# cxy1997/3D_adapt_auto_driving

Hardware: AMD Instinct MI355X
Metric: KITTI scenes/s end-to-end eval_rcnn (joint RPN+RCNN, synthetic 16384-pt scenes) (higher is better)
Workload: dtype f32; 1 GPU; BASELINE.json configs[2]: full PointRCNN RPN+RCNN inference, default.yaml shapes, random-init weights, batch=8 synthetic KITTI scenes x 16384 pts per GPU per step; scene=synth.scenes (SURVEY 8d: uniform clutter + ground + 10 dense cars), parallelism=scene-sharded x1, one final all_gather of detections, detections_gathered=652455, batch_slots=14, look_ahead=12, steps_per_launch=2

## Files before the change

3d_adapt_auto_driving_amd/csrc/packed_layer.hip:

```cpp
#include "common.hpp"
#include <cstdlib>
#include "segmax.hpp"

namespace prcnn {

unsigned int *next_ticket(hipStream_t st);

typedef float f32x4 __attribute__((ext_vector_type(4)));
constexpr int PL_ROWS = 64;
constexpr int PL_LD = 128 + 4;

constexpr int PL_MAX_BATCH = 4;
struct PLProblem {
    const unsigned int *hdr; long rows_host; int K, N; const float *A; long lda; const float *W; const float *bias; int do_relu;
    float *out; long ldo; const unsigned int *rowinfo; const int *tilecloud; int m, out_col, n_store;
    int lds_pool;
    const float *addG; const int *addIdx; const float *addW; int add_n, add_m; long add_ldg;
};
struct PLBatch { PLProblem p[PL_MAX_BATCH]; };
struct PGProblem {
    int n, c1; const unsigned int *hdr; const float4 *rowdxyz; const float4 *P; const float4 *wxyz; const unsigned int *rowinfo;
    const int *tilecloud; float4 *out;
};
struct PGBatch { PGProblem p[PL_MAX_BATCH]; };

__global__ __launch_bounds__(256) void packed_gather_affine_kernel(const PGBatch bt)
{
    const PGProblem &pb = bt.p[blockIdx.z];
    const int n = pb.n, c1 = pb.c1;
    const unsigned int *__restrict__ hdr = pb.hdr;
    const float4 *__restrict__ rowdxyz = pb.rowdxyz;
    const float4 *__restrict__ P = pb.P;
    const float4 *__restrict__ wxyz = pb.wxyz;
    const unsigned int *__restrict__ rowinfo = pb.rowinfo;
    const int *__restrict__ tilecloud = pb.tilecloud;
    float4 *__restrict__ out = pb.out;
    const long t = blockIdx.x;
    if (t >= (long)hdr[0]) return;
    const int cloud = tilecloud[t];
    const int q4 = c1 / 4;
    const long pbase = (long)cloud * n;
    for (int e = threadIdx.x; e < PL_ROWS * q4; e += 256) {
        const int row = e / q4, q = e - row * q4;
        const int k = (int)(rowinfo[t * PL_ROWS + row] & 0xffffu);
        const float4 d = rowdxyz[t * PL_ROWS + row];
        const float dx = d.x, dy = d.y, dz = d.z;
        const float4 base = P[(pbase + k) * q4 + q];
        const float4 wx = wxyz[q], wy = wxyz[q4 + q], wz = wxyz[2 * q4 + q];
        const float4 v = affine_relu4(base, wx, wy, wz, dx, dy, dz);
        out[(t * PL_ROWS + row) * q4 + q] = v;
    }
}

#define PL_LOAD_W(dst, kk)                                                                              \
    _Pragma("unroll") for (int s = 0; s < 64; ++s)                                                      \
        dst[s] = __uint_as_float(__builtin_amdgcn_raw_buffer_load_b32(wrs, lane_off, (unsigned int)((kk) + s) * row_bytes, 0));
#define PL_LOAD_A(dst, kk)                                                                              \
    _Pragma("unroll") for (int i = 0; i < 8; ++i) {                                                     \
        long g = t * PL_ROWS + r0 + 8 * i;                                                              \
        if (g >= rows) g = rows - 1;    \
        dst[i] = *reinterpret_cast<const f32x4 *>(A + g * lda + (kk) + 4 * chunk);                     \
    }
#define PL_STORE_A(src)                                                                                 \
    _Pragma("unroll") for (int i = 0; i < 8; ++i)                                                       \
        *reinterpret_cast<f32x4 *>(tile + (r0 + 8 * i) * PL_LD + 4 * chunk) = src[i];
#define PL_VM_DRAIN __builtin_amdgcn_s_waitcnt(0x0F70);
#define PL_GROUP_MFMA_HEAD(wf)                                                                          \
    acc0 = __builtin_amdgcn_mfma_f32_32x32x2f32(a0.x, wf[4 * g + 0], acc0, 0, 0, 0);                    \
    acc1 = __builtin_amdgcn_mfma_f32_32x32x2f32(a1.x, wf[4 * g + 0], acc1, 0, 0, 0);
#define PL_GROUP_MFMA_TAIL(wf)                                                                          \
    acc0 = __builtin_amdgcn_mfma_f32_32x32x2f32(a0.y, wf[4 * g + 1], acc0, 0, 0, 0);                    \
    acc1 = __builtin_amdgcn_mfma_f32_32x32x2f32(a1.y, wf[4 * g + 1], acc1, 0, 0, 0);                    \
    acc0 = __builtin_amdgcn_mfma_f32_32x32x2f32(a0.z, wf[4 * g + 2], acc0, 0, 0, 0);                    \
    acc1 = __builtin_amdgcn_mfma_f32_32x32x2f32(a1.z, wf[4 * g + 2], acc1, 0, 0, 0);                    \
    acc0 = __builtin_amdgcn_mfma_f32_32x32x2f32(a0.w, wf[4 * g + 3], acc0, 0, 0, 0);                    \
    acc1 = __builtin_amdgcn_mfma_f32_32x32x2f32(a1.w, wf[4 * g + 3], acc1, 0, 0, 0);
#define PL_STAGE(T, wf)                                                                                 \
    {                                                                                                   \
        const float *a0p = (T) + j * PL_LD + 64 * h, *a1p = (T) + (32 + j) * PL_LD + 64 * h;            \
        f32x4 a0 = *reinterpret_cast<const f32x4 *>(a0p);                                               \
        f32x4 a1 = *reinterpret_cast<const f32x4 *>(a1p);                                               \
        _Pragma("unroll") for (int g = 0; g < 16; ++g) {                                                \
            f32x4 n0 = a0, n1 = a1;                                                                     \
            if (g < 15) {                                                                               \
                n0 = *reinterpret_cast<const f32x4 *>(a0p + 4 * (g + 1));                               \
                n1 = *reinterpret_cast<const f32x4 *>(a1p + 4 * (g + 1));                               \
            }                                                                                           \
            __builtin_amdgcn_sched_barrier(0);                                                          \
            PL_GROUP_MFMA_HEAD(wf)                                                                      \
            PL_GROUP_MFMA_TAIL(wf)                                                                      \
            a0 = n0; a1 = n1;                                                                           \
        }                                                                                               \
    }
#define PL_SADD(x, y) asm volatile("s_add_u32 %0, %0, %1" : "+s"(x) : "s"(y) : "scc");
#define PL_STAGE_PREFETCH_X(T, TN, wf, wn, kn, ARS, LOFF)                                               \
    {                                                                                                   \
        const float *a0p = (T) + j * PL_LD + 64 * h, *a1p = (T) + (32 + j) * PL_LD + 64 * h;            \
        f32x4 a0 = *reinterpret_cast<const f32x4 *>(a0p);                                               \
        f32x4 a1 = *reinterpret_cast<const f32x4 *>(a1p);                                               \
        f32x4 ar[8];                                                                                    \
// ... 39 lines not shown
            __builtin_amdgcn_sched_barrier(0);                                                          \
            PL_GROUP_MFMA_HEAD(wf)                                                                      \
            if (g < 8)                                                                                  \
                ar[g] = __builtin_bit_cast(f32x4, __builtin_amdgcn_raw_buffer_load_b128(                \
                    ars, a_lane, (soff) + (unsigned int)(8 * g) * a_row_bytes, 0));                     \
            else                                                                                        \
                *reinterpret_cast<f32x4 *>((TN) + (r0 + 8 * (g - 8)) * PL_LD + 4 * chunk) = ar[g - 8];  \
            __builtin_amdgcn_sched_barrier(0);                                                          \
            PL_GROUP_MFMA_TAIL(wf)                                                                      \
            a0 = n0_; a1 = n1_;                                                                         \
        }                                                                                               \
    }

template <bool SEGMAX>
__device__ __forceinline__ void pl_epilogue(const f32x16 &acc0, const f32x16 &acc1, float *tile, int *ctr, long t, long rows, int n0,
                                            const float *__restrict__ bias, int do_relu, float *__restrict__ out, long ldo,
                                            const unsigned int *__restrict__ rowinfo, const int *__restrict__ tilecloud, int m,
                                            int out_col, int n_store, int lds_pool, const PLProblem *add = nullptr)
{
    const int tid = threadIdx.x, lane = tid & 63, w = tid >> 6, j = lane & 31, h = lane >> 5;
    const int chunk = tid & 31, r0 = tid >> 5;
    const float bcol = bias[n0 + 32 * w + j];
    if constexpr (SEGMAX) {
        if (tid < PL_ROWS) {
            const unsigned int info = rowinfo[t * PL_ROWS + tid];
            ctr[tid] = tilecloud[t] * m + (int)(info >> 16);
        }
        __syncthreads();
        const int myc = ctr[lane], prevc = ctr[lane ? lane - 1 : 0];
        const unsigned long long start = __ballot(lane == 0 || myc != prevc);
        if (!lds_pool || __popcll(start) <= PK_LDS_MIN) {
            pk_segmented_max(acc0, acc1, ctr, start, h, out, (int)ldo, out_col + n0 + 32 * w + j, bcol);
        } else {
            const float4 bias4 = *reinterpret_cast<const float4 *>(bias + n0 + 4 * chunk);
            pk_park(acc0, acc1, tile, PL_LD, 32 * w + j, h);
            lds_barrier();
            pk_segmented_max_lds(tile, PL_LD, ctr, tid, out, (int)ldo, out_col + n0, bias4);
        }
    } else {
        const bool with_add = add && add->addG;
        __syncthreads();
#pragma unroll
        for (int r = 0; r < 16; ++r) {
            const int row = (r & 3) + 8 * (r >> 2) + 4 * h;
            const float v0 = acc0[r] + bcol, v1 = acc1[r] + bcol;
            tile[row * PL_LD + 32 * w + j] = (do_relu && !with_add) ? fmaxf(v0, 0.f) : v0;
            tile[(32 + row) * PL_LD + 32 * w + j] = (do_relu && !with_add) ? fmaxf(v1, 0.f) : v1;
        }
        __syncthreads();
#pragma unroll
        for (int i = 0; i < 8; ++i) {
            const int row = r0 + 8 * i;
            const long g = t * PL_ROWS + row;
            if (g < rows) {
                const int c0 = n0 + 4 * chunk;
                float4 v = *reinterpret_cast<const float4 *>(tile + row * PL_LD + 4 * chunk);
                if (with_add) {
                    const int *ix = add->addIdx + g * 3;
                    const float *wv = add->addW + g * 3;
                    const long cb = (g / add->add_n) * (long)add->add_m;
                    const float4 g0 = *reinterpret_cast<const float4 *>(add->addG + (cb + ix[0]) * add->add_ldg + c0);
                    const float4 g1 = *reinterpret_cast<const float4 *>(add->addG + (cb + ix[1]) * add->add_ldg + c0);
                    const float4 g2 = *reinterpret_cast<const float4 *>(add->addG + (cb + ix[2]) * add->add_ldg + c0);
                    const float w0 = wv[0], w1 = wv[1], w2 = wv[2];
                    v.x = __fadd_rn(v.x, __fadd_rn(__fadd_rn(__fmul_rn(w0, g0.x), __fmul_rn(w1, g1.x)), __fmul_rn(w2, g2.x)));
                    v.y = __fadd_rn(v.y, __fadd_rn(__fadd_rn(__fmul_rn(w0, g0.y), __fmul_rn(w1, g1.y)), __fmul_rn(w2, g2.y)));
                    v.z = __fadd_rn(v.z, __fadd_rn(__fadd_rn(__fmul_rn(w0, g0.z), __fmul_rn(w1, g1.z)), __fmul_rn(w2, g2.z)));
                    v.w = __fadd_rn(v.w, __fadd_rn(__fadd_rn(__fmul_rn(w0, g0.w), __fmul_rn(w1, g1.w)), __fmul_rn(w2, g2.w)));
                    if (do_relu) v = make_float4(fmaxf(v.x, 0.f), fmaxf(v.y, 0.f), fmaxf(v.z, 0.f), fmaxf(v.w, 0.f));
                }
                if (c0 + 4 <= n_store && (ldo & 3) == 0) {
                    *reinterpret_cast<float4 *>(out + g * ldo + c0) = v;
                } else {
                    const float e[4] = {v.x, v.y, v.z, v.w};
#pragma unroll
                    for (int q = 0; q < 4; ++q)
                        if (c0 + q < n_store) out[g * ldo + c0 + q] = e[q];
                }
            }
        }
    }
}

template <bool SEGMAX>
__global__ __launch_bounds__(256, 2) void packed_layer_kernel(
    const PLBatch bt)
{
    const PLProblem &pb = bt.p[blockIdx.z];
    const unsigned int *__restrict__ hdr = pb.hdr;
    const long rows_host = pb.rows_host;
    const int K = pb.K, N = pb.N;
    const float *__restrict__ A = pb.A;
    const long lda = pb.lda;
    const float *__restrict__ W = pb.W;
    const float *__restrict__ bias = pb.bias;
    const int do_relu = pb.do_relu;
    float *__restrict__ out = pb.out;
    const long ldo = pb.ldo;
    const unsigned int *__restrict__ rowinfo = pb.rowinfo;
    const int *__restrict__ tilecloud = pb.tilecloud;
    const int m = pb.m, out_col = pb.out_col, n_store = pb.n_store;
    __shared__ float tile[PL_ROWS * PL_LD];
    __shared__ int ctr[PL_ROWS];
    const long t = blockIdx.x;
    const long rows = hdr ? (long)hdr[0] * PL_ROWS : rows_host;
    const int n0 = blockIdx.y * 128;
    if (t * PL_ROWS >= rows || n0 >= n_store) return;
    const int tid = threadIdx.x, lane = tid & 63, w = tid >> 6, j = lane & 31, h = lane >> 5;
    const int chunk = tid & 31, r0 = tid >> 5;
    f32x16 acc0 = {0}, acc1 = {0};
    const __amdgpu_buffer_rsrc_t wrs = __builtin_amdgcn_make_buffer_rsrc((void *)W, 0, K * N * 4, 0x00020000);
    const unsigned int row_bytes = (unsigned int)N * 4u;
    const unsigned int lane_off = ((unsigned int)(64 * h) * (unsigned int)N + (unsigned int)(n0 + 32 * w + j)) * 4u;
    for (int k0 = 0; k0 < K; k0 += 128) {
        float wf[64];
        f32x4 ar[8];
        PL_LOAD_W(wf, k0)
        PL_LOAD_A(ar, k0)
        if (k0) __syncthreads();
        PL_STORE_A(ar)
        __syncthreads();
        PL_STAGE(tile, wf)
    }
    pl_epilogue<SEGMAX>(acc0, acc1, tile, ctr, t, rows, n0, bias, do_relu, out, ldo, rowinfo, tilecloud, m, out_col, n_store, pb.lds_pool, &pb);
}

template <bool SEGMAX>
__global__ __launch_bounds__(256, 2) void packed_layer_pipe_kernel(
    const PLBatch bt)
{
    const PLProblem &pb = bt.p[blockIdx.z];
    const unsigned int *__restrict__ hdr = pb.hdr;
    const long rows_host = pb.rows_host;
    const int K = pb.K, N = pb.N;
    const float *__restrict__ A = pb.A;
    const long lda = pb.lda;
    const float *__restrict__ W = pb.W;
    const float *__restrict__ bias = pb.bias;
    const int do_relu = pb.do_relu;
    float *__restrict__ out = pb.out;
    const long ldo = pb.ldo;
    const unsigned int *__restrict__ rowinfo = pb.rowinfo;
    const int *__restrict__ tilecloud = pb.tilecloud;
    const int m = pb.m, out_col = pb.out_col, n_store = pb.n_store;
    __shared__ float tiles[2 * PL_ROWS * PL_LD];
    __shared__ int ctr[PL_ROWS];
    const long t = blockIdx.x;
    const long rows = hdr ? (long)hdr[0] * PL_ROWS : rows_host;
    const int n0 = blockIdx.y * 128;
    if (t * PL_ROWS >= rows || n0 >= n_store) return;
    const int tid = threadIdx.x, lane = tid & 63, j = lane & 31, h = lane >> 5;
    const int w = __builtin_amdgcn_readfirstlane(tid >> 6);
    const int chunk = tid & 31, r0 = tid >> 5;
    f32x16 acc0 = {0}, acc1 = {0};
    const __amdgpu_buffer_rsrc_t wrs = __builtin_amdgcn_make_buffer_rsrc((void *)W, 0, K * N * 4, 0x00020000);
    const unsigned int row_bytes = (unsigned int)N * 4u;
    const unsigned int lane_off = ((unsigned int)(64 * h) * (unsigned int)N + (unsigned int)(n0 + 32 * w + j)) * 4u;
    const long left = rows - t * PL_ROWS;
    const unsigned int a_row_bytes = (unsigned int)lda * 4u;
    const __amdgpu_buffer_rsrc_t ars = __builtin_amdgcn_make_buffer_rsrc(
        (void *)(A + t * PL_ROWS * lda), 0, (int)((left < PL_ROWS ? left : PL_ROWS) * (long)a_row_bytes), 0x00020000);
    const unsigned int a_lane = (unsigned int)r0 * a_row_bytes + 16u * chunk;
    float wa[64], wb[64];
    {
        PL_LOAD_W(wa, 0)
#pragma unroll
        for (int i = 0; i < 8; ++i)
            *reinterpret_cast<f32x4 *>(tiles + (r0 + 8 * i) * PL_LD + 4 * chunk) =
                __builtin_bit_cast(f32x4, __builtin_amdgcn_raw_buffer_load_b128(ars, a_lane, (unsigned int)(8 * i) * a_row_bytes, 0));
    }
    const int np = K >> 7;
    for (int p = 0; p < np; ++p) {
        PL_VM_DRAIN
        lds_barrier();
        const float *T = tiles + (p & 1) * (PL_ROWS * PL_LD);
        float *TN = tiles + ((p + 1) & 1) * (PL_ROWS * PL_LD);
        if (p + 1 < np) {
            PL_STAGE_PREFETCH(T, TN, wa, wb, (p + 1) * 128)
#pragma unroll
            for (int s = 0; s < 64; ++s) wa[s] = wb[s];
        } else {
            PL_STAGE(T, wa)
        }
    }
    if constexpr (!SEGMAX) {
        if (n0 + 128 <= n_store && !pb.addG) {
            const float bcol = bias[n0 + 32 * w + j];
            const unsigned int o_row_bytes = (unsigned int)ldo * 4u;
            const __amdgpu_buffer_rsrc_t ors = __builtin_amdgcn_make_buffer_rsrc(
                (void *)(out + t * PL_ROWS * ldo), 0, (int)((left < PL_ROWS ? left : PL_ROWS) * (long)o_row_bytes), 0x00020000);
            const unsigned int o_lane = (unsigned int)(4 * h) * o_row_bytes + (unsigned int)(n0 + 32 * w + j) * 4u;
#pragma unroll
            for (int r = 0; r < 16; ++r) {
                const unsigned int so = (unsigned int)((r & 3) + 8 * (r >> 2)) * o_row_bytes;
                const float v0 = acc0[r] + bcol, v1 = acc1[r] + bcol;
                __builtin_amdgcn_raw_buffer_store_b32(__float_as_uint(do_relu ? fmaxf(v0, 0.f) : v0), ors, o_lane, so, 0);
                __builtin_amdgcn_raw_buffer_store_b32(__float_as_uint(do_relu ? fmaxf(v1, 0.f) : v1), ors, o_lane, so + 32u * o_row_bytes, 0);
            }
            return;
        }
    }
    pl_epilogue<SEGMAX>(acc0, acc1, tiles, ctr, t, rows, n0, bias, do_relu, out, ldo, rowinfo, tilecloud, m, out_col, n_store, pb.lds_pool, &pb);
}

template <bool ADD>
__global__ __launch_bounds__(256, 2) void packed_layer_persist_kernel(
    long rows, int K, int N, const float *__restrict__ A, long lda, const float *__restrict__ W, const float *__restrict__ bias,
    int do_relu, float *__restrict__ out, long ldo, unsigned int *__restrict__ ticket, const PLProblem addp)
{
    __shared__ float tiles[2 * PL_ROWS * PL_LD];
    __shared__ unsigned int s_item[2];
    const int tid = threadIdx.x, lane = tid & 63, j = lane & 31, h = lane >> 5;
    const int w = __builtin_amdgcn_readfirstlane(tid >> 6);
    const int chunk = tid & 31, r0 = tid >> 5;
    const unsigned int col_blocks = (unsigned int)(N >> 7);
    const unsigned int n_tiles = (unsigned int)((rows + PL_ROWS - 1) / PL_ROWS);
    const unsigned int n_items = n_tiles * col_blocks;
    const __amdgpu_buffer_rsrc_t wrs = __builtin_amdgcn_make_buffer_rsrc((void *)W, 0, K * N * 4, 0x00020000);
    const unsigned int row_bytes = (unsigned int)N * 4u;
    const unsigned int a_row_bytes = (unsigned int)lda * 4u;
    const unsigned int a_lane = (unsigned int)r0 * a_row_bytes + 16u * chunk;
    const int np = K >> 7;
    auto tile_rsrc = [&](unsigned int t) __attribute__((always_inline)) {
        const long left = rows - (long)t * PL_ROWS;
        return __builtin_amdgcn_make_buffer_rsrc((void *)(A + (long)t * PL_ROWS * lda), 0,
                                                 (int)((left < PL_ROWS ? left : PL_ROWS) * (long)a_row_bytes), 0x00020000);
    };
    auto loff = [&](unsigned int cb) __attribute__((always_inline)) {
        return ((unsigned int)(64 * h) * (unsigned int)N + (cb * 128u + (unsigned int)(32 * w + j))) * 4u;
    };
    unsigned int item = blockIdx.x;
    unsigned int t = item / col_blocks, cb = item - t * col_blocks;
    __amdgpu_buffer_rsrc_t ars = tile_rsrc(t);
    unsigned int lane_off = loff(cb);
    float wa[64], wb[64];
    {
        PL_LOAD_W(wa, 0)
#pragma unroll
        for (int i = 0; i < 8; ++i)
            *reinterpret_cast<f32x4 *>(tiles + (r0 + 8 * i) * PL_LD + 4 * chunk) =
                __builtin_bit_cast(f32x4, __builtin_amdgcn_raw_buffer_load_b128(ars, a_lane, (unsigned int)(8 * i) * a_row_bytes, 0));
    }
    int pp = 0;
    int slot = 1;
    PL_VM_DRAIN
    while (true) {
        f32x16 acc0 = {0}, acc1 = {0};
        unsigned int next = 0xffffffffu, tn = 0, cbn = 0, drawn = 0;
        const float bcol = bias[(int)cb * 128 + 32 * w + j];
        for (int p = 0; p < np; ++p, ++pp) {
            if (p > 0) {
                PL_VM_DRAIN
                if (p == 1 && tid == 0) s_item[slot] = drawn;
            }
            lds_barrier();
            if (p == 0 && tid == 0) drawn = gridDim.x + atomicAdd(ticket, 1u);
            const float *T = tiles + (pp & 1) * (PL_ROWS * PL_LD);
            float *TN = tiles + ((pp + 1) & 1) * (PL_ROWS * PL_LD);
            if (p + 1 < np) {
                PL_STAGE_PREFETCH(T, TN, wa, wb, (p + 1) * 128)
#pragma unroll
                for (int s2 = 0; s2 < 64; ++s2) wa[s2] = wb[s2];
            } else {
                next = s_item[slot];
                if (next < n_items) {
                    tn = next / col_blocks; cbn = next - tn * col_blocks;
                    const __amdgpu_buffer_rsrc_t ars_n = tile_rsrc(tn);
                    const unsigned int loff_n = loff(cbn);
                    PL_STAGE_PREFETCH_X(T, TN, wa, wb, 0, ars_n, loff_n)
#pragma unroll
                    for (int s2 = 0; s2 < 64; ++s2) wa[s2] = wb[s2];
                    PL_VM_DRAIN
                } else {
                    PL_STAGE(T, wa)
                }
            }
        }
        if constexpr (ADD) {
            float *Tlast = tiles + ((pp - 1) & 1) * (PL_ROWS * PL_LD);
            pl_epilogue<false>(acc0, acc1, Tlast, nullptr, (long)t, rows, (int)cb * 128, bias, do_relu, out, ldo, nullptr, nullptr, 0, 0, N, 0, &addp);
            __syncthreads();
        } else {
            const long left = rows - (long)t * PL_ROWS;
            const unsigned int o_row_bytes = (unsigned int)ldo * 4u;
            const __amdgpu_buffer_rsrc_t ors = __builtin_amdgcn_make_buffer_rsrc(
                (void *)(out + (long)t * PL_ROWS * ldo), 0, (int)((left < PL_ROWS ? left : PL_ROWS) * (long)o_row_bytes), 0x00020000);
            const unsigned int o_lane = (unsigned int)(4 * h) * o_row_bytes + (cb * 128u + (unsigned int)(32 * w + j)) * 4u;
#pragma unroll
            for (int r = 0; r < 16; ++r) {
                const unsigned int so = (unsigned int)((r & 3) + 8 * (r >> 2)) * o_row_bytes;
                const float v0 = acc0[r] + bcol, v1 = acc1[r] + bcol;
                __builtin_amdgcn_raw_buffer_store_b32(__float_as_uint(do_relu ? fmaxf(v0, 0.f) : v0), ors, o_lane, so, 0);
                __builtin_amdgcn_raw_buffer_store_b32(__float_as_uint(do_relu ? fmaxf(v1, 0.f) : v1), ors, o_lane, so + 32u * o_row_bytes, 0);
            }
        }
        if (next >= n_items) break;
        t = tn; cb = cbn;
        ars = tile_rsrc(t);
        lane_off = loff(cb);
        slot ^= 1;
    }
    if (tid == 0) ticket_release(ticket);
}

__global__ __launch_bounds__(256, 2) void packed_layer_stream_kernel(long rows, int N, const float *__restrict__ A, long lda,
                                                                     const float *__restrict__ W, const float *__restrict__ bias,
                                                                     int do_relu, float *__restrict__ out, long ldo, int n_store,
                                                                     const PLProblem addp )
{
    __shared__ float tiles[2 * PL_ROWS * PL_LD];
    const int tid = threadIdx.x, lane = tid & 63, j = lane & 31, h = lane >> 5;
    const int w = __builtin_amdgcn_readfirstlane(tid >> 6);
    const int chunk = tid & 31, r0 = tid >> 5;
    const int n0 = blockIdx.y * 128;
    const long ntiles = (rows + PL_ROWS - 1) / PL_ROWS;
    long t = blockIdx.x;
    if (t >= ntiles || n0 >= n_store) return;
    const __amdgpu_buffer_rsrc_t wrs = __builtin_amdgcn_make_buffer_rsrc((void *)W, 0, 128 * N * 4, 0x00020000);
    const unsigned int row_bytes = (unsigned int)N * 4u;
    const unsigned int lane_off = ((unsigned int)(64 * h) * (unsigned int)N + (unsigned int)(n0 + 32 * w + j)) * 4u;
    float wf[64];
    PL_LOAD_W(wf, 0)
    const unsigned int a_row_bytes = (unsigned int)lda * 4u;
    const __amdgpu_buffer_rsrc_t ars = __builtin_amdgcn_make_buffer_rsrc((void *)A, 0, (int)(rows * (long)a_row_bytes), 0x00020000);
    const unsigned int a_lane = (unsigned int)r0 * a_row_bytes + 16u * chunk;
    {
        const unsigned int soff = (unsigned int)(t * PL_ROWS) * a_row_bytes;
#pragma unroll
        for (int i = 0; i < 8; ++i)
            *reinterpret_cast<f32x4 *>(tiles + (r0 + 8 * i) * PL_LD + 4 * chunk) =
                __builtin_bit_cast(f32x4, __builtin_amdgcn_raw_buffer_load_b128(ars, a_lane, soff + (unsigned int)(8 * i) * a_row_bytes, 0));
    }
    const float bcol = bias[n0 + 32 * w + j];
    const bool direct = n0 + 128 <= n_store && !addp.addG;
    const unsigned int o_row_bytes = (unsigned int)ldo * 4u;
    const unsigned int o_lane = (unsigned int)(4 * h) * o_row_bytes + (unsigned int)(n0 + 32 * w + j) * 4u;
    PL_VM_DRAIN
    for (int it = 0;; ++it) {
        lds_barrier();
        float *T = tiles + (it & 1) * (PL_ROWS * PL_LD);
        float *TN = tiles + ((it + 1) & 1) * (PL_ROWS * PL_LD);
        const long tn = t + gridDim.x;
        f32x16 acc0 = {0}, acc1 = {0};
        if (tn < ntiles) {
            const unsigned int soff = (unsigned int)(tn * PL_ROWS) * a_row_bytes;
            PL_STAGE_ROWS(T, TN, wf, soff)
        } else {
            PL_STAGE(T, wf)
        }
        if (direct) {
            const long left = rows - t * PL_ROWS;
            const __amdgpu_buffer_rsrc_t ors = __builtin_amdgcn_make_buffer_rsrc(
                (void *)(out + t * PL_ROWS * ldo), 0, (int)((left < PL_ROWS ? left : PL_ROWS) * (long)o_row_bytes), 0x00020000);
#pragma unroll
            for (int r = 0; r < 16; ++r) {
                const unsigned int so = (unsigned int)((r & 3) + 8 * (r >> 2)) * o_row_bytes;
                const float v0 = acc0[r] + bcol, v1 = acc1[r] + bcol;
                __builtin_amdgcn_raw_buffer_store_b32(__float_as_uint(do_relu ? fmaxf(v0, 0.f) : v0), ors, o_lane, so, 0);
                __builtin_amdgcn_raw_buffer_store_b32(__float_as_uint(do_relu ? fmaxf(v1, 0.f) : v1), ors, o_lane, so + 32u * o_row_bytes, 0);
            }
        } else {
            pl_epilogue<false>(acc0, acc1, T, nullptr, t, rows, n0, bias, do_relu, out, ldo, nullptr, nullptr, 0, 0, n_store, 0, &addp);
            __syncthreads();
        }
        if (tn >= ntiles) break;
        t = tn;
    }
}

#define PL32_GROUP(wf, BODY)                                                                            \
    acc = __builtin_amdgcn_mfma_f32_32x32x2f32(a.x, wf[4 * g + 0], acc, 0, 0, 0);                       \
    BODY                                                                                                \
    __builtin_amdgcn_sched_barrier(0);                                                                  \
    acc = __builtin_amdgcn_mfma_f32_32x32x2f32(a.y, wf[4 * g + 1], acc, 0, 0, 0);                       \
    acc = __builtin_amdgcn_mfma_f32_32x32x2f32(a.z, wf[4 * g + 2], acc, 0, 0, 0);                       \
    acc = __builtin_amdgcn_mfma_f32_32x32x2f32(a.w, wf[4 * g + 3], acc, 0, 0, 0);
__global__ __launch_bounds__(256, 2) void packed_layer_pipe32_kernel(const PLBatch bt)
{
    const PLProblem &pb = bt.p[blockIdx.z];
    const long rows = pb.rows_host;
    const int K = pb.K, N = pb.N;
    const float *__restrict__ A = pb.A;
    const long lda = pb.lda;
// ... 145 lines not shown

extern "C" int prcnn_packed_gather_affine_batch(int nprob, const prcnn_gather_problem *pr, void *stream)
{
    PRCNN_REQUIRE(nprob >= 0 && nprob <= PL_MAX_BATCH && (nprob == 0 || pr), "packed_gather_affine: 0..%d problems", PL_MAX_BATCH);
    PGBatch bt;
    int k = 0;
    long grid_x = 0;
    for (int i = 0; i < nprob; ++i) {
        const prcnn_gather_problem &q = pr[i];
        PRCNN_REQUIRE(q.b >= 0 && q.n >= 0 && q.max_tiles >= 0 && q.c1 > 0 && q.c1 % 4 == 0, "packed_gather_affine: bad sizes");
        if (q.max_tiles == 0) continue;
        PRCNN_REQUIRE(q.P && q.wxyz && q.rowinfo && q.rowdxyz && q.tilecloud && q.hdr && q.out, "packed_gather_affine: null pointer");
        PRCNN_REQUIRE((((uintptr_t)q.P | (uintptr_t)q.wxyz | (uintptr_t)q.out) & 15) == 0, "packed_gather_affine: 16-byte alignment required");
        PRCNN_REQUIRE(q.max_tiles <= 0x7fffffffL, "packed_gather_affine: too many tiles");
        bt.p[k++] = PGProblem{q.n, q.c1, q.hdr, (const float4 *)q.rowdxyz, (const float4 *)q.P, (const float4 *)q.wxyz, q.rowinfo,
                              q.tilecloud, (float4 *)q.out};
        if (q.max_tiles > grid_x) grid_x = q.max_tiles;
    }
    if (k == 0) return PRCNN_OK;
    hipLaunchKernelGGL(packed_gather_affine_kernel, dim3((unsigned)grid_x, 1, k), dim3(256), 0, (hipStream_t)stream, bt);
    return check_launch("packed_gather_affine");
}

extern "C" int prcnn_packed_gather_affine(int b, int n, int c1, long max_tiles, const float *P, const float *wxyz,
                                          const unsigned int *rowinfo, const float *rowdxyz, const int *tilecloud,
                                          const unsigned int *hdr, float *out, void *stream)
{
    const prcnn_gather_problem q = {b, n, c1, max_tiles, P, wxyz, rowinfo, rowdxyz, tilecloud, hdr, out};
    return prcnn_packed_gather_affine_batch(1, &q, stream);
}

namespace {
enum PLClass { PL_ONE, PL_PIPE, PL_PIPE32, PL_STREAM };
}
extern "C" int prcnn_packed_layer_batch(int nprob, const prcnn_layer_problem *pr, int segmax, void *stream)
{
    PRCNN_REQUIRE(nprob >= 0 && nprob <= PL_MAX_BATCH && (nprob == 0 || pr), "packed_layer: 0..%d problems", PL_MAX_BATCH);
    hipStream_t st = (hipStream_t)stream;
    PLBatch bt;
    PLClass cls[PL_MAX_BATCH];
    long tiles_of[PL_MAX_BATCH];
    int blocks_of[PL_MAX_BATCH], src[PL_MAX_BATCH];
    int k = 0;
    for (int i = 0; i < nprob; ++i) {
        const prcnn_layer_problem &q = pr[i];
        PRCNN_REQUIRE(q.K > 0 && q.N > 0 && q.K % 128 == 0 && q.N % 128 == 0, "packed_layer: K=%d, N=%d must be multiples of 128", q.K, q.N);
        PRCNN_REQUIRE(q.lda >= q.K && q.lda % 4 == 0, "packed_layer: bad leading dimension of A");
        long tiles;
        int n_store;
        if (segmax) {
            PRCNN_REQUIRE(q.b >= 0 && q.m >= 0 && q.max_tiles >= 0 && q.out_col >= 0 && q.ldo >= q.out_col + q.N, "packed_layer_segmax: bad layout");
            if ((long)q.b * q.m == 0) continue;
            PRCNN_REQUIRE(q.A && q.W && q.bias && q.rowinfo && q.tilecloud && q.hdr && q.out, "packed_layer_segmax: null pointer");
            PRCNN_REQUIRE(((uintptr_t)q.A & 15) == 0 && q.max_tiles <= 0x7fffffffL, "packed_layer_segmax: alignment / size");
            if (!q.out_is_zero && hipMemset2DAsync(q.out + q.out_col, (size_t)q.ldo * sizeof(float), 0, (size_t)q.N * sizeof(float),
                                                    (size_t)q.b * q.m, st) != hipSuccess) {
                set_error("packed_layer_segmax: cannot zero the output slice");
                return PRCNN_ELAUNCH;
            }
            tiles = q.max_tiles;
            n_store = q.N;
        } else {
            PRCNN_REQUIRE(q.n_store >= 1 && q.n_store <= q.N && q.ldo >= q.n_store, "packed_layer: n_store=%d outside 1..N (or ldo too small)", q.n_store);
            tiles = q.hdr ? q.max_tiles : (q.rows + PL_ROWS - 1) / PL_ROWS;
            PRCNN_REQUIRE(tiles >= 0 && tiles <= 0x7fffffffL && q.rows >= 0, "packed_layer: bad row count");
            n_store = q.n_store;
            if (tiles > 0) {
                PRCNN_REQUIRE(q.A && q.W && q.bias && q.out, "packed_layer: null pointer");
                PRCNN_REQUIRE(((uintptr_t)q.A & 15) == 0 && (((uintptr_t)q.out & 15) == 0 || (q.ldo & 3) != 0), "packed_layer: 16-byte alignment required");
            }
        }
        if (tiles == 0) continue;
        const int col_blocks = (n_store + 127) / 128;
        const bool pipe = q.K >= 256 && pipe_enabled();
        cls[k] = (!segmax && !q.hdr && pipe && tiles * col_blocks < 256) ? PL_PIPE32 : (pipe ? PL_PIPE : PL_ONE);
        if (cls[k] == PL_ONE && !segmax && !q.hdr && q.K == 128 && tiles * col_blocks >= stream_min() && stream_enabled() &&
            q.rows * q.lda * 4 < (1L << 31))
            cls[k] = PL_STREAM;
        tiles_of[k] = tiles; blocks_of[k] = col_blocks; src[k] = i;
        bt.p[k] = PLProblem{q.hdr, q.rows, q.K, q.N, q.A, q.lda, q.W, q.bias, segmax ? 1 : q.relu, q.out, q.ldo,
                            segmax ? q.rowinfo : nullptr, segmax ? q.tilecloud : nullptr, segmax ? q.m : 0, segmax ? q.out_col : 0, n_store,
                            (segmax && segmax_lds_enabled() && (((uintptr_t)q.out | (uintptr_t)q.bias) & 15) == 0 && (q.ldo & 3) == 0 &&
                             (q.out_col & 3) == 0) ? 1 : 0,
                            nullptr, nullptr, nullptr, 0, 0, 0};
        ++k;
    }
    if (k == 0) return PRCNN_OK;
    const bool persist = true;
    if (persist && k == 1 && cls[0] == PL_PIPE && !segmax && !bt.p[0].hdr && bt.p[0].n_store == bt.p[0].N && !pr[src[0]].hdr &&
        tiles_of[0] * blocks_of[0] > stream_cap() && tiles_of[0] * blocks_of[0] >= persist_min()) {
        const PLProblem &q = bt.p[0];
        const long items = tiles_of[0] * blocks_of[0];
        const long cap = stream_cap();
        unsigned int *ticket = next_ticket(st);
        if (!ticket) { set_error("packed_layer: cannot set up the item ticket"); return PRCNN_ELAUNCH; }
        hipLaunchKernelGGL(packed_layer_persist_kernel<false>, dim3((unsigned)(items < cap ? items : cap)), dim3(256), 0, st, q.rows_host, q.K, q.N,
                           q.A, q.lda, q.W, q.bias, q.do_relu, q.out, q.ldo, ticket, PLProblem{});
        return check_launch("packed_layer");
    }
    bool together = cls[0] != PL_STREAM;
    for (int i = 1; i < k; ++i) together = together && cls[i] == cls[0];
    if (together && cls[0] == PL_PIPE32) {
        long gx = 0;
        int gy = 0;
        for (int r = 0; r < k; ++r) {
            const long t32 = (bt.p[r].rows_host + 31) / 32;
            if (t32 > gx) gx = t32;
            if (blocks_of[r] > gy) gy = blocks_of[r];
        }
        hipLaunchKernelGGL(packed_layer_pipe32_kernel, dim3((unsigned)gx, gy, k), dim3(256), 0, st, bt);
        return check_launch("packed_layer");
    }
    for (int i = 0; i < k; ++i) {
        PLBatch one;
        long gx = tiles_of[i];
        int gy = blocks_of[i], gz = 1;
        if (together) {
            for (int r = 1; r < k; ++r) { if (tiles_of[r] > gx) gx = tiles_of[r]; if (blocks_of[r] > gy) gy = blocks_of[r]; }
            gz = k;
        } else {
            one.p[0] = bt.p[i];
        }
        const PLBatch &arg = together ? bt : one;
        if (cls[i] == PL_STREAM) {
            const prcnn_layer_problem &q = pr[src[i]];
            const long cap = stream_cap() / gy > 0 ? stream_cap() / gy : 1;
            hipLaunchKernelGGL(packed_layer_stream_kernel, dim3((unsigned)(tiles_of[i] < cap ? tiles_of[i] : cap), gy), dim3(256), 0, st,
                               q.rows, q.N, q.A, q.lda, q.W, q.bias, q.relu, q.out, q.ldo, q.n_store, PLProblem{});
        } else if (cls[i] == PL_PIPE32) {
            const prcnn_layer_problem &q = pr[src[i]];
            hipLaunchKernelGGL(packed_layer_pipe32_kernel, dim3((unsigned)((q.rows + 31) / 32), gy), dim3(256), 0, st, one);
        } else if (segmax) {
            auto kern = cls[i] == PL_PIPE ? packed_layer_pipe_kernel<true> : packed_layer_kernel<true>;
            hipLaunchKernelGGL(kern, dim3((unsigned)gx, gy, gz), dim3(256), 0, st, arg);
        } else {
            auto kern = cls[i] == PL_PIPE ? packed_layer_pipe_kernel<false> : packed_layer_kernel<false>;
            hipLaunchKernelGGL(kern, dim3((unsigned)gx, gy, gz), dim3(256), 0, st, arg);
        }
        const int rc = check_launch(segmax ? "packed_layer_segmax" : "packed_layer");
        if (rc != PRCNN_OK || together) return rc;
    }
    return PRCNN_OK;
}

extern "C" int prcnn_packed_layer(const unsigned int *hdr, long rows, long max_tiles, int K, int N, int n_store, const float *A,
                                  long lda, const float *W, const float *bias, int relu, float *out, long ldo, void *stream)
{
    prcnn_layer_problem q = {};
    q.hdr = hdr; q.rows = rows; q.max_tiles = max_tiles; q.K = K; q.N = N; q.n_store = n_store; q.A = A; q.lda = lda; q.W = W;
    q.bias = bias; q.relu = relu; q.out = out; q.ldo = ldo;
    return prcnn_packed_layer_batch(1, &q, 0, stream);
}

extern "C" int prcnn_packed_layer_segmax(int b, int m, long max_tiles, int K, int N, const float *A, long lda, const float *W,
                                         const float *bias, const unsigned int *rowinfo, const int *tilecloud,
                                         const unsigned int *hdr, float *out, int out_stride, int out_col, int out_is_zero, void *stream)
{
    prcnn_layer_problem q = {};
    q.hdr = hdr; q.max_tiles = max_tiles; q.K = K; q.N = N; q.n_store = N; q.A = A; q.lda = lda; q.W = W; q.bias = bias; q.relu = 1;
    q.out = out; q.ldo = out_stride; q.b = b; q.m = m; q.rowinfo = rowinfo; q.tilecloud = tilecloud; q.out_col = out_col;
    q.out_is_zero = out_is_zero;
    return prcnn_packed_layer_batch(1, &q, 1, stream);
}


extern "C" int prcnn_packed_layer_interp(long rows, int K, int N, const float *A, long lda, const float *W, const float *bias, int relu,
                                         float *out, long ldo, int n_per_cloud, int m_known, const float *G, long ldg, const int *idx,
                                         const float *weight, void *stream)
{
    PRCNN_REQUIRE(rows >= 0 && K > 0 && N > 0 && K % 128 == 0 && N % 128 == 0, "packed_layer_interp: K=%d, N=%d must be multiples of 128", K, N);
    PRCNN_REQUIRE(lda >= K && lda % 4 == 0 && ldo >= N && ldo % 4 == 0 && ldg >= N && ldg % 4 == 0, "packed_layer_interp: bad leading dimensions");
    PRCNN_REQUIRE(n_per_cloud >= 1 && m_known >= 1 && rows % n_per_cloud == 0, "packed_layer_interp: rows must be whole clouds");
    if (rows == 0) return PRCNN_OK;
    PRCNN_REQUIRE(A && W && bias && out && G && idx && weight, "packed_layer_interp: null pointer");
    PRCNN_REQUIRE((((uintptr_t)A | (uintptr_t)out | (uintptr_t)G) & 15) == 0, "packed_layer_interp: 16-byte alignment required");
    const long tiles = (rows + PL_ROWS - 1) / PL_ROWS;
    PRCNN_REQUIRE(tiles <= 0x7fffffffL, "packed_layer_interp: too many rows");
    PLBatch bt;
    bt.p[0] = PLProblem{nullptr, rows, K, N, A, lda, W, bias, relu, out, ldo, nullptr, nullptr, 0, 0, N, 0,
                        G, idx, weight, n_per_cloud, m_known, ldg};
    const bool persist = true;
    const long items = tiles * (N / 128);
    hipStream_t st = (hipStream_t)stream;
    if (persist && K == 128 && stream_enabled() && items >= stream_min() && rows * lda * 4 < (1L << 31)) {
        const long cap = stream_cap() / (N / 128) > 0 ? stream_cap() / (N / 128) : 1;
        hipLaunchKernelGGL(packed_layer_stream_kernel, dim3((unsigned)(tiles < cap ? tiles : cap), N / 128), dim3(256), 0, st, rows, N, A, lda,
                           W, bias, relu, out, ldo, N, bt.p[0]);
        return check_launch("packed_layer_interp");
    }
    if (persist && K >= 256 && pipe_enabled() && items > stream_cap() && items >= persist_min()) {
        const long cap = stream_cap();
        unsigned int *ticket = next_ticket(st);
        if (!ticket) { set_error("packed_layer_interp: cannot set up the item ticket"); return PRCNN_ELAUNCH; }
        hipLaunchKernelGGL(packed_layer_persist_kernel<true>, dim3((unsigned)(items < cap ? items : cap)), dim3(256), 0, st, rows, K, N, A, lda,
                           W, bias, relu, out, ldo, ticket, bt.p[0]);
        return check_launch("packed_layer_interp");
    }
    auto kern = (K >= 256 && pipe_enabled()) ? packed_layer_pipe_kernel<false> : packed_layer_kernel<false>;
    hipLaunchKernelGGL(kern, dim3((unsigned)tiles, N / 128, 1), dim3(256), 0, st, bt);
    return check_launch("packed_layer_interp");
}
```

Measured before the change: 8647 scenes/s.

## Add persistent work-queue kernel for batched packed layers with cross-item prefetch

Adds a persistent packed_layer_queue_kernel that flattens every (problem, tile, column-block) item of a batched layer launch into one atomic-ticket queue. Each block prefetches the next item's weights and activations while finishing the current one. The dispatcher routes batched PIPE/ONE problems, segmax layers, and device-sized (hdr) problems through this queue instead of a padded 3-D grid sized to the largest problem. The goal is to remove empty blocks spent on dead tiles, cut launch overhead, and hide the load stall at tile boundaries. The cost is a ticket atomic, per-item decode work, and more register pressure.

```diff
diff --git a/3d_adapt_auto_driving_amd/csrc/packed_layer.hip b/3d_adapt_auto_driving_amd/csrc/packed_layer.hip
--- a/3d_adapt_auto_driving_amd/csrc/packed_layer.hip
+++ b/3d_adapt_auto_driving_amd/csrc/packed_layer.hip
@@ -16,6 +16,7 @@
     float *out; long ldo; const unsigned int *rowinfo; const int *tilecloud; int m, out_col, n_store;
     int lds_pool;
     const float *addG; const int *addIdx; const float *addW; int add_n, add_m; long add_ldg;
+    long max_tiles;
 };
 struct PLBatch { PLProblem p[PL_MAX_BATCH]; };
 struct PGProblem {
@@ -221,7 +222,6 @@
     }
 }
 
-template <bool SEGMAX>
 __global__ __launch_bounds__(256, 2) void packed_layer_kernel(
     const PLBatch bt)
 {
@@ -240,7 +240,6 @@
     const int *__restrict__ tilecloud = pb.tilecloud;
     const int m = pb.m, out_col = pb.out_col, n_store = pb.n_store;
     __shared__ float tile[PL_ROWS * PL_LD];
-    __shared__ int ctr[PL_ROWS];
     const long t = blockIdx.x;
     const long rows = hdr ? (long)hdr[0] * PL_ROWS : rows_host;
     const int n0 = blockIdx.y * 128;
@@ -261,10 +260,9 @@
         __syncthreads();
         PL_STAGE(tile, wf)
     }
-    pl_epilogue<SEGMAX>(acc0, acc1, tile, ctr, t, rows, n0, bias, do_relu, out, ldo, rowinfo, tilecloud, m, out_col, n_store, pb.lds_pool, &pb);
-}
-
-template <bool SEGMAX>
+    pl_epilogue<false>(acc0, acc1, tile, nullptr, t, rows, n0, bias, do_relu, out, ldo, rowinfo, tilecloud, m, out_col, n_store, pb.lds_pool, &pb);
+}
+
 __global__ __launch_bounds__(256, 2) void packed_layer_pipe_kernel(
     const PLBatch bt)
 {
@@ -283,7 +281,6 @@
     const int *__restrict__ tilecloud = pb.tilecloud;
     const int m = pb.m, out_col = pb.out_col, n_store = pb.n_store;
     __shared__ float tiles[2 * PL_ROWS * PL_LD];
-    __shared__ int ctr[PL_ROWS];
     const long t = blockIdx.x;
     const long rows = hdr ? (long)hdr[0] * PL_ROWS : rows_host;
     const int n0 = blockIdx.y * 128;
@@ -322,7 +319,7 @@
             PL_STAGE(T, wa)
         }
     }
-    if constexpr (!SEGMAX) {
+    {
         if (n0 + 128 <= n_store && !pb.addG) {
             const float bcol = bias[n0 + 32 * w + j];
             const unsigned int o_row_bytes = (unsigned int)ldo * 4u;
@@ -339,7 +336,7 @@
             return;
         }
     }
-    pl_epilogue<SEGMAX>(acc0, acc1, tiles, ctr, t, rows, n0, bias, do_relu, out, ldo, rowinfo, tilecloud, m, out_col, n_store, pb.lds_pool, &pb);
+    pl_epilogue<false>(acc0, acc1, tiles, nullptr, t, rows, n0, bias, do_relu, out, ldo, rowinfo, tilecloud, m, out_col, n_store, pb.lds_pool, &pb);
 }
 
 template <bool ADD>
@@ -438,6 +435,152 @@
         ars = tile_rsrc(t);
         lane_off = loff(cb);
         slot ^= 1;
+    }
+    if (tid == 0) ticket_release(ticket);
+}
+
+template <bool SEGMAX>
+__global__ __launch_bounds__(256, 2) void packed_layer_queue_kernel(const PLBatch bt, const int nprob, unsigned int *__restrict__ ticket)
+{
+    __shared__ float tiles[2 * PL_ROWS * PL_LD];
+    __shared__ int ctr[PL_ROWS];
+    __shared__ unsigned int s_item[2];
+    const int tid = threadIdx.x, lane = tid & 63, j = lane & 31, h = lane >> 5;
+    const int w = __builtin_amdgcn_readfirstlane(tid >> 6);
+    const int chunk = tid & 31, r0 = tid >> 5;
+    unsigned int ends[PL_MAX_BATCH], cbs[PL_MAX_BATCH], total = 0;
+#pragma unroll
+    for (int p = 0; p < PL_MAX_BATCH; ++p) {
+        unsigned int tl = 0, cbk = 1;
+        if (p < nprob) {
+            const PLProblem &q = bt.p[p];
+            if (q.hdr) {
+                const unsigned int live = q.hdr[0], room = (unsigned int)q.max_tiles;
+                tl = live < room ? live : room;
+            } else {
+                tl = (unsigned int)((q.rows_host + PL_ROWS - 1) / PL_ROWS);
+            }
+            cbk = (unsigned int)(q.n_store + 127) >> 7;
+        }
+        total += tl * cbk;
+        ends[p] = total; cbs[p] = cbk;
+    }
+    unsigned int cur = blockIdx.x, nxt = gridDim.x + blockIdx.x;
+    if (cur >= total) {
+        if (tid == 0) ticket_release(ticket);
+        return;
+    }
+    auto decode = [&](unsigned int item, int &p, unsigned int &t, unsigned int &cb) __attribute__((always_inline)) {
+        unsigned int start = 0, cbk = cbs[0];
+        p = 0;
+#pragma unroll
+        for (int q = 1; q < PL_MAX_BATCH; ++q)
+            if (item >= ends[q - 1]) { p = q; start = ends[q - 1]; cbk = cbs[q]; }
+        const unsigned int local = item - start;
+        t = local / cbk; cb = local - t * cbk;
+    };
+    auto context = [&](int p, unsigned int t, unsigned int cb, __amdgpu_buffer_rsrc_t &wrs_, __amdgpu_buffer_rsrc_t &ars_,
+                       unsigned int &rb_, unsigned int &arb_, unsigned int &alane_, unsigned int &loff_, int &np_) __attribute__((always_inline)) {
+        const PLProblem &q = bt.p[p];
+        const long left = q.hdr ? (long)PL_ROWS : q.rows_host - (long)t * PL_ROWS;
+        wrs_ = __builtin_amdgcn_make_buffer_rsrc((void *)q.W, 0, q.K * q.N * 4, 0x00020000);
+        rb_ = (unsigned int)q.N * 4u;
+        arb_ = (unsigned int)q.lda * 4u;
+        ars_ = __builtin_amdgcn_make_buffer_rsrc((void *)(q.A + (long)t * PL_ROWS * q.lda), 0,
+                                                 (int)((left < PL_ROWS ? left : PL_ROWS) * (long)arb_), 0x00020000);
+        alane_ = (unsigned int)r0 * arb_ + 16u * chunk;
+        loff_ = ((unsigned int)(64 * h) * (unsigned int)q.N + (cb * 128u + (unsigned int)(32 * w + j))) * 4u;
+        np_ = q.K >> 7;
+    };
+    int pc, c_np;
+    unsigned int t, cb, c_rb, c_arb, c_alane, c_loff;
+    __amdgpu_buffer_rsrc_t c_wrs, c_ars;
+    decode(cur, pc, t, cb);
+    context(pc, t, cb, c_wrs, c_ars, c_rb, c_arb, c_alane, c_loff, c_np);
+    float wa[64], wb[64];
+    {
+        const __amdgpu_buffer_rsrc_t wrs = c_wrs;
+        const unsigned int row_bytes = c_rb, lane_off = c_loff;
+        PL_LOAD_W(wa, 0)
+#pragma unroll
+        for (int i = 0; i < 8; ++i)
+            *reinterpret_cast<f32x4 *>(tiles + (r0 + 8 * i) * PL_LD + 4 * chunk) =
+                __builtin_bit_cast(f32x4, __builtin_amdgcn_raw_buffer_load_b128(c_ars, c_alane, (unsigned int)(8 * i) * c_arb, 0));
+    }
+    int pp = 0;
+    unsigned int it = 0;
+    PL_VM_DRAIN
+    while (true) {
+        f32x16 acc0 = {0}, acc1 = {0};
+        unsigned int drawn = 0, tn = 0, cbn = 0, n_rb = 0, n_arb = 0, n_alane = 0, n_loff = 0;
+        int pn = 0, n_np = 0;
+        __amdgpu_buffer_rsrc_t n_wrs = c_wrs, n_ars = c_ars;
+        bool have_next = false;
+        const PLProblem &qc = bt.p[pc];
+        float bcol = 0.f;
+        if constexpr (!SEGMAX) bcol = qc.bias[(int)cb * 128 + 32 * w + j];
+        for (int p = 0; p < c_np; ++p, ++pp) {
+            if (p > 0) PL_VM_DRAIN
+            lds_barrier();
+            if (p == 0) {
+                if (it > 0) nxt = (unsigned int)__builtin_amdgcn_readfirstlane((int)s_item[(it - 1) & 1]);
+                if (tid == 0) drawn = 2u * gridDim.x + atomicAdd(ticket, 1u);
+            }
+            const float *T = tiles + (pp & 1) * (PL_ROWS * PL_LD);
+            float *TN = tiles + ((pp + 1) & 1) * (PL_ROWS * PL_LD);
+            const bool last = p + 1 == c_np;
+            if (!last || nxt < total) {
+                __amdgpu_buffer_rsrc_t f_wrs = c_wrs, f_ars = c_ars;
+                unsigned int f_rb = c_rb, f_arb = c_arb, f_alane = c_alane, f_loff = c_loff, f_kn = (unsigned int)(p + 1) * 128u;
+                if (last) {
+                    decode(nxt, pn, tn, cbn);
+                    context(pn, tn, cbn, n_wrs, n_ars, n_rb, n_arb, n_alane, n_loff, n_np);
+                    f_wrs = n_wrs; f_ars = n_ars; f_rb = n_rb; f_arb = n_arb; f_alane = n_alane; f_loff = n_loff; f_kn = 0;
+                    have_next = true;
+                }
+                {
+                    const __amdgpu_buffer_rsrc_t wrs = f_wrs;
+                    const unsigned int row_bytes = f_rb, a_row_bytes = f_arb, a_lane = f_alane;
+                    PL_STAGE_PREFETCH_X(T, TN, wa, wb, f_kn, f_ars, f_loff)
+                }
+#pragma unroll
+                for (int s2 = 0; s2 < 64; ++s2) wa[s2] = wb[s2];
+                if (last) PL_VM_DRAIN
+            } else {
+                PL_STAGE(T, wa)
+            }
+        }
+        if (tid == 0) s_item[it & 1] = drawn;
+        const int n0 = (int)cb * 128;
+        const long rows_c = qc.hdr ? ((long)t + 1) * PL_ROWS : qc.rows_host;
+        float *Tlast = tiles + ((pp - 1) & 1) * (PL_ROWS * PL_LD);
+        if constexpr (SEGMAX) {
+            pl_epilogue<true>(acc0, acc1, Tlast, ctr, (long)t, rows_c, n0, qc.bias, 1, qc.out, qc.ldo, qc.rowinfo, qc.tilecloud, qc.m,
+                              qc.out_col, qc.n_store, qc.lds_pool);
+            __syncthreads();
+        } else if (n0 + 128 <= qc.n_store) {
+            const long left = rows_c - (long)t * PL_ROWS;
+            const unsigned int o_row_bytes = (unsigned int)qc.ldo * 4u;
+            const int do_relu = qc.do_relu;
+            const __amdgpu_buffer_rsrc_t ors = __builtin_amdgcn_make_buffer_rsrc(
+                (void *)(qc.out + (long)t * PL_ROWS * qc.ldo), 0, (int)((left < PL_ROWS ? left : PL_ROWS) * (long)o_row_bytes), 0x00020000);
+            const unsigned int o_lane = (unsigned int)(4 * h) * o_row_bytes + (cb * 128u + (unsigned int)(32 * w + j)) * 4u;
+#pragma unroll
+            for (int r = 0; r < 16; ++r) {
+                const unsigned int so = (unsigned int)((r & 3) + 8 * (r >> 2)) * o_row_bytes;
+                const float v0 = acc0[r] + bcol, v1 = acc1[r] + bcol;
+                __builtin_amdgcn_raw_buffer_store_b32(__float_as_uint(do_relu ? fmaxf(v0, 0.f) : v0), ors, o_lane, so, 0);
+                __builtin_amdgcn_raw_buffer_store_b32(__float_as_uint(do_relu ? fmaxf(v1, 0.f) : v1), ors, o_lane, so + 32u * o_row_bytes, 0);
+            }
+        } else {
+            pl_epilogue<false>(acc0, acc1, Tlast, nullptr, (long)t, rows_c, n0, qc.bias, qc.do_relu, qc.out, qc.ldo, nullptr, nullptr, 0, 0,
+                               qc.n_store, 0);
+            __syncthreads();
+        }
+        if (!have_next) break;
+        pc = pn; t = tn; cb = cbn; c_np = n_np;
+        c_wrs = n_wrs; c_ars = n_ars; c_rb = n_rb; c_arb = n_arb; c_alane = n_alane; c_loff = n_loff;
+        ++it;
     }
     if (tid == 0) ticket_release(ticket);
 }
@@ -749,7 +892,7 @@
                             segmax ? q.rowinfo : nullptr, segmax ? q.tilecloud : nullptr, segmax ? q.m : 0, segmax ? q.out_col : 0, n_store,
                             (segmax && segmax_lds_enabled() && (((uintptr_t)q.out | (uintptr_t)q.bias) & 15) == 0 && (q.ldo & 3) == 0 &&
                              (q.out_col & 3) == 0) ? 1 : 0,
-                            nullptr, nullptr, nullptr, 0, 0, 0};
+                            nullptr, nullptr, nullptr, 0, 0, 0, q.hdr ? tiles : 0};
         ++k;
     }
     if (k == 0) return PRCNN_OK;
@@ -765,47 +908,63 @@
                            q.A, q.lda, q.W, q.bias, q.do_relu, q.out, q.ldo, ticket, PLProblem{});
         return check_launch("packed_layer");
     }
-    bool together = cls[0] != PL_STREAM;
-    for (int i = 1; i < k; ++i) together = together && cls[i] == cls[0];
-    if (together && cls[0] == PL_PIPE32) {
-        long gx = 0;
-        int gy = 0;
-        for (int r = 0; r < k; ++r) {
-            const long t32 = (bt.p[r].rows_host + 31) / 32;
-            if (t32 > gx) gx = t32;
-            if (blocks_of[r] > gy) gy = blocks_of[r];
-        }
-        hipLaunchKernelGGL(packed_layer_pipe32_kernel, dim3((unsigned)gx, gy, k), dim3(256), 0, st, bt);
-        return check_launch("packed_layer");
+    const auto queue_class = [&](int i) { return cls[i] == PL_PIPE || cls[i] == PL_ONE; };
+    const auto launch_queue = [&](const PLBatch &arg, int n, long items) -> int {
+        if (items > 0x7fffffffL - 4 * stream_cap()) { set_error("packed_layer: too many (tile, column block) items"); return PRCNN_EINVAL; }
+        const long cap = stream_cap() > 0 ? stream_cap() : 1;
+        unsigned int *ticket = next_ticket(st);
+        if (!ticket) { set_error("packed_layer: cannot set up the item ticket"); return PRCNN_ELAUNCH; }
+        const dim3 grid((unsigned)(items < cap ? items : cap));
+        if (segmax)
+            hipLaunchKernelGGL(packed_layer_queue_kernel<true>, grid, dim3(256), 0, st, arg, n, ticket);
+        else
+            hipLaunchKernelGGL(packed_layer_queue_kernel<false>, grid, dim3(256), 0, st, arg, n, ticket);
+        return check_launch(segmax ? "packed_layer_segmax" : "packed_layer");
+    };
+    const auto wants_queue = [&](int i) {
+        return queue_class(i) && (segmax || bt.p[i].hdr || tiles_of[i] * blocks_of[i] > stream_cap());
+    };
+    if (k > 1) {
+        bool all_queue = true;
+        long items = 0;
+        for (int i = 0; i < k; ++i) { all_queue = all_queue && queue_class(i); items += tiles_of[i] * blocks_of[i]; }
+        if (all_queue) return launch_queue(bt, k, items);
+        bool all32 = true;
+        for (int i = 0; i < k; ++i) all32 = all32 && cls[i] == PL_PIPE32;
+        if (all32) {
+            long gx = 0;
+            int gy = 0;
+            for (int r = 0; r < k; ++r) {
+                const long t32 = (bt.p[r].rows_host + 31) / 32;
+                if (t32 > gx) gx = t32;
+                if (blocks_of[r] > gy) gy = blocks_of[r];
+            }
+            hipLaunchKernelGGL(packed_layer_pipe32_kernel, dim3((unsigned)gx, gy, k), dim3(256), 0, st, bt);
+            return check_launch("packed_layer");
+        }
     }
     for (int i = 0; i < k; ++i) {
         PLBatch one;
-        long gx = tiles_of[i];
-        int gy = blocks_of[i], gz = 1;
-        if (together) {
-            for (int r = 1; r < k; ++r) { if (tiles_of[r] > gx) gx = tiles_of[r]; if (blocks_of[r] > gy) gy = blocks_of[r]; }
-            gz = k;
+        one.p[0] = bt.p[i];
+        const int gy = blocks_of[i];
+        int rc;
+        if (wants_queue(i)) {
+            rc = launch_queue(one, 1, tiles_of[i] * blocks_of[i]);
         } else {
-            one.p[0] = bt.p[i];
-        }
-        const PLBatch &arg = together ? bt : one;
-        if (cls[i] == PL_STREAM) {
             const prcnn_layer_problem &q = pr[src[i]];
-            const long cap = stream_cap() / gy > 0 ? stream_cap() / gy : 1;
-            hipLaunchKernelGGL(packed_layer_stream_kernel, dim3((unsigned)(tiles_of[i] < cap ? tiles_of[i] : cap), gy), dim3(256), 0, st,
-                               q.rows, q.N, q.A, q.lda, q.W, q.bias, q.relu, q.out, q.ldo, q.n_store, PLProblem{});
-        } else if (cls[i] == PL_PIPE32) {
-            const prcnn_layer_problem &q = pr[src[i]];
-            hipLaunchKernelGGL(packed_layer_pipe32_kernel, dim3((unsigned)((q.rows + 31) / 32), gy), dim3(256), 0, st, one);
-        } else if (segmax) {
-            auto kern = cls[i] == PL_PIPE ? packed_layer_pipe_kernel<true> : packed_layer_kernel<true>;
-            hipLaunchKernelGGL(kern, dim3((unsigned)gx, gy, gz), dim3(256), 0, st, arg);
-        } else {
-            auto kern = cls[i] == PL_PIPE ? packed_layer_pipe_kernel<false> : packed_layer_kernel<false>;
-            hipLaunchKernelGGL(kern, dim3((unsigned)gx, gy, gz), dim3(256), 0, st, arg);
-        }
-        const int rc = check_launch(segmax ? "packed_layer_segmax" : "packed_layer");
-        if (rc != PRCNN_OK || together) return rc;
+            if (cls[i] == PL_STREAM) {
+                const long cap = stream_cap() / gy > 0 ? stream_cap() / gy : 1;
+                hipLaunchKernelGGL(packed_layer_stream_kernel, dim3((unsigned)(tiles_of[i] < cap ? tiles_of[i] : cap), gy), dim3(256), 0, st,
+                                   q.rows, q.N, q.A, q.lda, q.W, q.bias, q.relu, q.out, q.ldo, q.n_store, PLProblem{});
+            } else if (cls[i] == PL_PIPE32) {
+                hipLaunchKernelGGL(packed_layer_pipe32_kernel, dim3((unsigned)((q.rows + 31) / 32), gy), dim3(256), 0, st, one);
+            } else {
+                auto kern = cls[i] == PL_PIPE ? packed_layer_pipe_kernel : packed_layer_kernel;
+                hipLaunchKernelGGL(kern, dim3((unsigned)tiles_of[i], gy, 1), dim3(256), 0, st, one);
+            }
+            rc = check_launch("packed_layer");
+        }
+        if (rc != PRCNN_OK) return rc;
     }
     return PRCNN_OK;
 }
@@ -863,7 +1022,7 @@
                            W, bias, relu, out, ldo, ticket, bt.p[0]);
         return check_launch("packed_layer_interp");
     }
-    auto kern = (K >= 256 && pipe_enabled()) ? packed_layer_pipe_kernel<false> : packed_layer_kernel<false>;
+    auto kern = (K >= 256 && pipe_enabled()) ? packed_layer_pipe_kernel : packed_layer_kernel;
     hipLaunchKernelGGL(kern, dim3((unsigned)tiles, N / 128, 1), dim3(256), 0, st, bt);
     return check_launch("packed_layer_interp");
 }
```

Measured after the change: 8694 scenes/s (median of 6 runs). About the same (+0.5%).
